# nextpyp/cet_pick

Hardware: AMD Instinct MI355X
Metric: subtomograms/sec (MoCo-3D train) + voxels/sec (heatmap+NMS) at 1/2/4/8 GPU (higher is better)
Workload: dtype f32; 1 GPU; moco_main.py moco3d_18: 3D encoder, synthetic 512x512x128 tomogram, 32^3 subtomo crops, batch 64 per GPU, r=1024, dim=128, m=0.999, T=0.1, SGD lr 1e-3; global_batch=64, parallelism=dp1, hipgraph=True

## Files before the change

### cet_pick_amd/csrc/train_ops.hip

```cpp
#include "common.h"
#include "bf16x3.h"
#include <algorithm>

namespace {

using bf3::ld4;
using bf3::st4;

enum { CR_STATS = 0, CR_BNBWD = 1, CR_SUM = 2, CR_BNBWD_X = 3 };

struct PoolGeom { int N, Di, Hi, Wi, Do, Ho, Wo, k, s, pad; };

struct ColReduceParams {
    const float* a;
    const float* x;
    const float* y;
    const float* save;
    long M;
    int C, relu;
    double* partials;
    const float* gamma;
    const float* beta;
    double* sums_direct;
    float* f32_direct;
// ... 41 lines not shown
            float4 x4 = ld4(p.x + o);
            float x[4] = {x4.x, x4.y, x4.z, x4.w};
            if (p.relu) {
                float4 y4 = ld4(p.y + o);
                float y[4] = {y4.x, y4.y, y4.z, y4.w};
#pragma unroll
                for (int i = 0; i < 4; ++i) a[i] = y[i] > 0.f ? a[i] : 0.f;
            }
#pragma unroll
            for (int i = 0; i < 4; ++i) { s0[i] += a[i]; s1[i] = fmaf(a[i], (x[i] - mean[i]) * inv[i], s1[i]); }
        } else {
#pragma unroll
            for (int i = 0; i < 4; ++i) s0[i] += a[i];
        }
    }
    __shared__ double red[2][256][4];
#pragma unroll
    for (int i = 0; i < 4; ++i) {
        red[0][threadIdx.x][i] = MODE == CR_STATS ? w0[i] : (double)s0[i];
        red[1][threadIdx.x][i] = MODE == CR_STATS ? w1[i] : (double)s1[i];
    }
    __syncthreads();
    if (trow == 0) {
        double a0[4] = {0, 0, 0, 0}, a1[4] = {0, 0, 0, 0};
        for (int rr = 0; rr < RS; ++rr)
#pragma unroll
            for (int i = 0; i < 4; ++i) { a0[i] += red[0][rr * CV + tcol][i]; a1[i] += red[1][rr * CV + tcol][i]; }
        double* dst = p.sums_direct ? p.sums_direct : p.partials + (long)blockIdx.x * 2 * p.C;
#pragma unroll
        for (int i = 0; i < 4; ++i) {
            dst[4 * tcol + i] = a0[i]; dst[p.C + 4 * tcol + i] = a1[i];
            if (p.f32_direct) {
                if (4 * tcol + i < p.n_f32) p.f32_direct[4 * tcol + i] = (float)a0[i];
                if (p.C + 4 * tcol + i < p.n_f32) p.f32_direct[p.C + 4 * tcol + i] = (float)a1[i];
            }
        }
    }
}

__global__ __launch_bounds__(256) void colreduce_finalize_kernel(const double* partials, int n_part,
                                                                int C, double* sums, float* sums_f32, int n_f32) {
    const int c = blockIdx.x * 8 + (threadIdx.x >> 5), l = threadIdx.x & 31;
    double s = 0;
    if (c < 2 * C) {
        int b = l;
        for (; b + 7 * 32 < n_part; b += 8 * 32) {
            double v[8];
#pragma unroll
            for (int u = 0; u < 8; ++u) v[u] = partials[(long)(b + 32 * u) * 2 * C + c];
#pragma unroll
            for (int u = 0; u < 8; ++u) s += v[u];
        }
        for (; b < n_part; b += 32) s += partials[(long)b * 2 * C + c];
    }
#pragma unroll
    for (int o = 16; o > 0; o >>= 1) s += __shfl_xor(s, o, 32);
    if (l == 0 && c < 2 * C) {
        sums[c] = s;
        if (sums_f32 && c < n_f32) sums_f32[c] = (float)s;
    }
}

int colreduce_blocks(long M, int C) {
    int RS = 256 / (C / 4);
    long b = (M + (long)RS * 8 - 1) / ((long)RS * 8);
    long cap = 512;
    if (const char* v = getenv("MI_COLREDUCE_BLOCKS")) { const long cv = atol(v); if (cv >= 1 && cv <= 4096) cap = cv; }
    return (int)std::max<long>(1, std::min<long>(b, cap));
}
bool colreduce_ok(int C) { return C >= 4 && (C % 4) == 0 && (C / 4) <= 256 && (256 % (C / 4)) == 0; }

template <int MODE>
int run_colreduce(ColReduceParams p, double* sums, void* ws, size_t ws_bytes, hipStream_t s, float* sums_f32 = nullptr,
                  int n_f32 = 0) {
    if (!colreduce_ok(p.C) || p.M <= 0) return MI_E_ARG;
    int blocks = colreduce_blocks(p.M, p.C);
    if (!ws || ws_bytes < sizeof(double) * 2 * p.C * (size_t)blocks) return MI_E_WORKSPACE;
    p.partials = (double*)ws;
    if (blocks == 1) {
        p.sums_direct = sums; p.f32_direct = sums_f32; p.n_f32 = n_f32;
        hipLaunchKernelGGL((colreduce_kernel<MODE>), dim3(1), dim3(256), 0, s, p);
        MI_RETURN_IF_LAUNCH_FAILED();
        return MI_OK;
    }
    hipLaunchKernelGGL((colreduce_kernel<MODE>), dim3(blocks), dim3(256), 0, s, p);
    MI_RETURN_IF_LAUNCH_FAILED();
    hipLaunchKernelGGL(colreduce_finalize_kernel, dim3((2 * p.C + 7) / 8), dim3(256), 0, s,
                       (const double*)ws, blocks, p.C, sums, sums_f32, n_f32);
    MI_RETURN_IF_LAUNCH_FAILED();
    return MI_OK;
}

struct BnStat4 { float mean[4], inv[4]; double var[4]; };
__device__ __forceinline__ BnStat4 bn_stat4(const double* sums, double count, int C, int c, float eps) {
    BnStat4 r;
#pragma unroll
    for (int k = 0; k < 4; ++k) {
        const double mean = sums[c + k] / count;
        double var = sums[C + c + k] / count - mean * mean;
        if (var < 0) var = 0;
        r.mean[k] = (float)mean;
        r.inv[k] = (float)(1.0 / sqrt(var + (double)eps));
        r.var[k] = var;
    }
    return r;
}

__global__ __launch_bounds__(256) void bn_apply_kernel(const float* x, float* y, long n4, int C,
                                                      const double* sums, double count, float eps,
                                                      float momentum, float* running_mean,
                                                      float* running_var, long long* num_batches_tracked,
                                                      float* save, const float* gamma,
                                                      const float* beta, const float* res, int relu) {
    const int CV = C >> 2;
    const int c = (int)(threadIdx.x % CV) * 4;
    float m[4], iv[4];
    if (sums) {
        const BnStat4 st = bn_stat4(sums, count, C, c, eps);
#pragma unroll
        for (int k = 0; k < 4; ++k) { m[k] = st.mean[k]; iv[k] = st.inv[k]; }
        if (blockIdx.x == 0 && threadIdx.x < CV) {
#pragma unroll
            for (int k = 0; k < 4; ++k) {
                if (save) { save[c + k] = m[k]; save[C + c + k] = iv[k]; }
                if (running_mean) {
                    const double unbiased = count > 1 ? st.var[k] * count / (count - 1.0) : st.var[k];
                    running_mean[c + k] = (1.f - momentum) * running_mean[c + k] + momentum * m[k];
                    running_var[c + k] = (1.f - momentum) * running_var[c + k] + momentum * (float)unbiased;
                }
            }
            if (threadIdx.x == 0 && num_batches_tracked) *num_batches_tracked += 1;
        }
    } else {
#pragma unroll
        for (int k = 0; k < 4; ++k) { m[k] = running_mean[c + k]; iv[k] = 1.0f / sqrtf(running_var[c + k] + eps); }
        if (save && blockIdx.x == 0 && threadIdx.x < CV) {
#pragma unroll
            for (int k = 0; k < 4; ++k) { save[c + k] = m[k]; save[C + c + k] = iv[k]; }
        }
    }
    const float4 g = gamma ? ld4(gamma + c) : make_float4(1, 1, 1, 1);
    const float4 b = beta ? ld4(beta + c) : make_float4(0, 0, 0, 0);
    for (long i = (long)blockIdx.x * 256 + threadIdx.x; i < n4; i += (long)gridDim.x * 256) {
        float4 v = ld4(x + 4 * i);
        float4 o;
        o.x = fmaf((v.x - m[0]) * iv[0], g.x, b.x); o.y = fmaf((v.y - m[1]) * iv[1], g.y, b.y);
        o.z = fmaf((v.z - m[2]) * iv[2], g.z, b.z); o.w = fmaf((v.w - m[3]) * iv[3], g.w, b.w);
        if (res) { float4 r = ld4(res + 4 * i); o.x += r.x; o.y += r.y; o.z += r.z; o.w += r.w; }
        if (relu) { o.x = fmaxf(o.x, 0.f); o.y = fmaxf(o.y, 0.f); o.z = fmaxf(o.z, 0.f); o.w = fmaxf(o.w, 0.f); }
        st4(y + 4 * i, o);
    }
}

__global__ __launch_bounds__(256) void bn_relu_maxpool_fwd_kernel(const float* x, float* y, uint8_t* arg, PoolGeom g,
                                                                 int C, const double* sums, double count, float eps,
                                                                 float momentum, float* running_mean,
                                                                 float* running_var, long long* num_batches_tracked,
                                                                 float* save, const float* gamma, const float* beta) {
    const int CV = C >> 2;
    const int c = (int)(threadIdx.x % CV) * 4;
    float m[4], iv[4];
    if (sums) {
        const BnStat4 st = bn_stat4(sums, count, C, c, eps);
#pragma unroll
        for (int k = 0; k < 4; ++k) { m[k] = st.mean[k]; iv[k] = st.inv[k]; }
        if (blockIdx.x == 0 && threadIdx.x < CV) {
#pragma unroll
            for (int k = 0; k < 4; ++k) {
                if (save) { save[c + k] = m[k]; save[C + c + k] = iv[k]; }
                if (running_mean) {
                    const double unbiased = count > 1 ? st.var[k] * count / (count - 1.0) : st.var[k];
                    running_mean[c + k] = (1.f - momentum) * running_mean[c + k] + momentum * m[k];
                    running_var[c + k] = (1.f - momentum) * running_var[c + k] + momentum * (float)unbiased;
                }
            }
            if (threadIdx.x == 0 && num_batches_tracked) *num_batches_tracked += 1;
        }
    } else {
#pragma unroll
        for (int k = 0; k < 4; ++k) { m[k] = running_mean[c + k]; iv[k] = 1.0f / sqrtf(running_var[c + k] + eps); }
    }
    const float4 g4 = gamma ? ld4(gamma + c) : make_float4(1, 1, 1, 1);
    const float4 b4 = beta ? ld4(beta + c) : make_float4(0, 0, 0, 0);
    const float gg[4] = {g4.x, g4.y, g4.z, g4.w}, bb[4] = {b4.x, b4.y, b4.z, b4.w};
    const long total = (long)g.N * g.Do * g.Ho * g.Wo * CV;
    for (long i = (long)blockIdx.x * 256 + threadIdx.x; i < total; i += (long)gridDim.x * 256) {
        unsigned v = (unsigned)i / (unsigned)CV;
        const int xo = (int)(v % (unsigned)g.Wo); v /= (unsigned)g.Wo;
        const int yo = (int)(v % (unsigned)g.Ho); v /= (unsigned)g.Ho;
        const int zo = (int)(v % (unsigned)g.Do);
        const int n = (int)(v / (unsigned)g.Do);
        float best[4] = {-INFINITY, -INFINITY, -INFINITY, -INFINITY};
        int bi[4] = {0, 0, 0, 0};
        bool first = true;
        if (g.k == 3) {
            for (int a = 0; a < 3; ++a) {
                const int zi = zo * g.s - g.pad + a;
                const bool zok = (unsigned)zi < (unsigned)g.Di;
                float4 t9[9];
                bool ok9[9];
#pragma unroll
                for (int q = 0; q < 9; ++q) {
                    const int yi = yo * g.s - g.pad + q / 3, xi = xo * g.s - g.pad + q % 3;
                    ok9[q] = zok & ((unsigned)yi < (unsigned)g.Hi) & ((unsigned)xi < (unsigned)g.Wi);
                    const int zc = min(max(zi, 0), g.Di - 1), yc = min(max(yi, 0), g.Hi - 1), xc = min(max(xi, 0), g.Wi - 1);
                    t9[q] = ld4(x + ((((long)n * g.Di + zc) * g.Hi + yc) * g.Wi + xc) * C + c);
                }
#pragma unroll
                for (int q = 0; q < 9; ++q) {
                    if (!ok9[q]) continue;
                    const float xv[4] = {t9[q].x, t9[q].y, t9[q].z, t9[q].w};
                    const int tap = a * 9 + q;
#pragma unroll
                    for (int r = 0; r < 4; ++r) {
                        const float t = fmaxf(fmaf((xv[r] - m[r]) * iv[r], gg[r], bb[r]), 0.f);
                        const float tn = xv[r] != xv[r] ? xv[r] : t;
                        if (first || tn > best[r] || tn != tn) { best[r] = tn; bi[r] = tap; }
                    }
                    first = false;
                }
            }
        } else
        for (int a = 0; a < g.k; ++a) {
            const int zi = zo * g.s - g.pad + a;
            if ((unsigned)zi >= (unsigned)g.Di) continue;
            for (int b = 0; b < g.k; ++b) {
                const int yi = yo * g.s - g.pad + b;
                if ((unsigned)yi >= (unsigned)g.Hi) continue;
                for (int cc = 0; cc < g.k; ++cc) {
                    const int xi = xo * g.s - g.pad + cc;
                    if ((unsigned)xi >= (unsigned)g.Wi) continue;
                    const float4 t4 = ld4(x + ((((long)n * g.Di + zi) * g.Hi + yi) * g.Wi + xi) * C + c);
                    const float xv[4] = {t4.x, t4.y, t4.z, t4.w};
                    const int tap = (a * g.k + b) * g.k + cc;
#pragma unroll
                    for (int q = 0; q < 4; ++q) {
                        const float t = fmaxf(fmaf((xv[q] - m[q]) * iv[q], gg[q], bb[q]), 0.f);
                        const float tn = xv[q] != xv[q] ? xv[q] : t;
                        if (first || tn > best[q] || tn != tn) { best[q] = tn; bi[q] = tap; }
                    }
                    first = false;
                }
            }
        }
        st4(y + 4 * i, make_float4(best[0], best[1], best[2], best[3]));
        if (arg) *reinterpret_cast<uchar4*>(arg + 4 * i) = make_uchar4(bi[0], bi[1], bi[2], bi[3]);
    }
}

__global__ __launch_bounds__(256) void bn_relu_bwd_apply_x_kernel(const float* dy, const float* x, float* dx, long n4, int C,
                                                                 const float* save, const float* gamma, const float* beta,
                                                                 const double* sums, double count, float* dgamma,
                                                                 float* dbeta) {
    const int CV = C >> 2;
    const int c = (int)(threadIdx.x % CV) * 4;
    const float rc = (float)(1.0 / count);
    float mean[4], inv[4], gi[4], gg[4], bb[4], sdy[4], sdx[4];
#pragma unroll
    for (int k = 0; k < 4; ++k) {
        mean[k] = save[c + k]; inv[k] = save[C + c + k];
        gg[k] = gamma ? gamma[c + k] : 1.f; bb[k] = beta ? beta[c + k] : 0.f;
        gi[k] = gg[k] * inv[k];
        sdy[k] = (float)sums[c + k] * rc; sdx[k] = (float)sums[C + c + k] * rc;
    }
    if (blockIdx.x == 0 && threadIdx.x < CV) {
#pragma unroll
        for (int k = 0; k < 4; ++k) {
            if (dbeta) dbeta[c + k] = (float)sums[c + k];
            if (dgamma) dgamma[c + k] = (float)sums[C + c + k];
        }
    }
    for (long i = (long)blockIdx.x * 256 + threadIdx.x; i < n4; i += (long)gridDim.x * 256) {
        const float4 d4 = ld4(dy + 4 * i), x4 = ld4(x + 4 * i);
        const float d[4] = {d4.x, d4.y, d4.z, d4.w}, xv[4] = {x4.x, x4.y, x4.z, x4.w};
        float o[4];
#pragma unroll
        for (int k = 0; k < 4; ++k) {
            const float xh = (xv[k] - mean[k]) * inv[k];
            const float dm = fmaf(xh, gg[k], bb[k]) > 0.f ? d[k] : 0.f;
            o[k] = gi[k] * (dm - sdy[k] - xh * sdx[k]);
        }
        st4(dx + 4 * i, make_float4(o[0], o[1], o[2], o[3]));
    }
}

constexpr int BNS_CH = 4;

__device__ __forceinline__ void bns_block_sum8(double (&v)[8], double (*red)[8]) {
#pragma unroll
    for (int k = 0; k < 8; ++k)
#pragma unroll
        for (int o = 32; o > 0; o >>= 1) v[k] += __shfl_xor(v[k], o, 64);
    const int wave = threadIdx.x >> 6;
    if ((threadIdx.x & 63) == 0)
#pragma unroll
        for (int k = 0; k < 8; ++k) red[wave][k] = v[k];
    __syncthreads();
#pragma unroll
    for (int k = 0; k < 8; ++k) v[k] = (red[0][k] + red[1][k]) + (red[2][k] + red[3][k]);
}

__global__ __launch_bounds__(256) void bn_small_fwd_kernel(const float* x, float* y, int M, int C, const float* gamma,
                                                          const float* beta, float eps, float momentum,
                                                          float* running_mean, float* running_var,
                                                          long long* num_batches_tracked, float* save,
                                                          const float* res, int relu, float* pooled, int V) {
    const int c = blockIdx.x * BNS_CH;
    __shared__ double red[4][8];
    double s[8] = {0, 0, 0, 0, 0, 0, 0, 0};
#pragma unroll 4
    for (int r = threadIdx.x; r < M; r += 256) {
        const float4 v = ld4(x + (long)r * C + c);
        const float a[4] = {v.x, v.y, v.z, v.w};
#pragma unroll
        for (int k = 0; k < 4; ++k) { s[k] += (double)a[k]; s[4 + k] += (double)a[k] * (double)a[k]; }
    }
    bns_block_sum8(s, red);
    float m[4], iv[4];
#pragma unroll
    for (int k = 0; k < 4; ++k) {
        const double mean = s[k] / M;
        double var = s[4 + k] / M - mean * mean;
        if (var < 0) var = 0;
        m[k] = (float)mean; iv[k] = (float)(1.0 / sqrt(var + (double)eps));
        if (threadIdx.x == 0) {
            if (save) { save[c + k] = m[k]; save[C + c + k] = iv[k]; }
            if (running_mean) {
                const double unbiased = M > 1 ? var * M / (M - 1.0) : var;
                running_mean[c + k] = (1.f - momentum) * running_mean[c + k] + momentum * m[k];
                running_var[c + k] = (1.f - momentum) * running_var[c + k] + momentum * (float)unbiased;
            }
        }
    }
    if (blockIdx.x == 0 && threadIdx.x == 0 && num_batches_tracked) *num_batches_tracked += 1;
    const float4 g = gamma ? ld4(gamma + c) : make_float4(1, 1, 1, 1);
    const float4 b = beta ? ld4(beta + c) : make_float4(0, 0, 0, 0);
    if (pooled) {
        const int lane = threadIdx.x & 63;
        for (int r0 = 0; r0 < M; r0 += 256) {
            const int r = r0 + threadIdx.x;
            const bool ok = r < M;
            const long o = (long)(ok ? r : 0) * C + c;
            const float4 v = ld4(x + o);
            float q[4];
            q[0] = fmaf((v.x - m[0]) * iv[0], g.x, b.x); q[1] = fmaf((v.y - m[1]) * iv[1], g.y, b.y);
            q[2] = fmaf((v.z - m[2]) * iv[2], g.z, b.z); q[3] = fmaf((v.w - m[3]) * iv[3], g.w, b.w);
            if (relu) { q[0] = fmaxf(q[0], 0.f); q[1] = fmaxf(q[1], 0.f); q[2] = fmaxf(q[2], 0.f); q[3] = fmaxf(q[3], 0.f); }
            if (ok) st4(y + o, make_float4(q[0], q[1], q[2], q[3]));
            float acc[4] = {q[0], q[1], q[2], q[3]};
            for (int k = 1; k < V; ++k)
#pragma unroll
                for (int e = 0; e < 4; ++e) acc[e] += __shfl(q[e], (lane & ~(V - 1)) + k, 64);
            if (ok && (lane & (V - 1)) == 0) {
                const float rs = (float)V;
                st4(pooled + (long)(r / V) * C + c, make_float4(acc[0] / rs, acc[1] / rs, acc[2] / rs, acc[3] / rs));
            }
        }
        return;
    }
#pragma unroll 4
    for (int r = threadIdx.x; r < M; r += 256) {
        const long o = (long)r * C + c;
        const float4 v = ld4(x + o);
        float4 q;
        q.x = fmaf((v.x - m[0]) * iv[0], g.x, b.x); q.y = fmaf((v.y - m[1]) * iv[1], g.y, b.y);
        q.z = fmaf((v.z - m[2]) * iv[2], g.z, b.z); q.w = fmaf((v.w - m[3]) * iv[3], g.w, b.w);
        if (res) { const float4 t = ld4(res + o); q.x += t.x; q.y += t.y; q.z += t.z; q.w += t.w; }
        if (relu) { q.x = fmaxf(q.x, 0.f); q.y = fmaxf(q.y, 0.f); q.z = fmaxf(q.z, 0.f); q.w = fmaxf(q.w, 0.f); }
        st4(y + o, q);
    }
}

__global__ __launch_bounds__(256) void bn_small_bwd_kernel(const float* dy, const float* x, const float* y, float* dx,
                                                          int M, int C, const float* save, const float* gamma,
                                                          int relu, float* dgamma, float* dbeta, int V) {
    const int c = blockIdx.x * BNS_CH;
    __shared__ double red[4][8];
    const float4 ma = ld4(save + c), ia = ld4(save + C + c);
    const float mean[4] = {ma.x, ma.y, ma.z, ma.w}, inv[4] = {ia.x, ia.y, ia.z, ia.w};
    double s[8] = {0, 0, 0, 0, 0, 0, 0, 0};
#pragma unroll 4
    for (int r = threadIdx.x; r < M; r += 256) {
        const long o = (long)r * C + c;
        const float4 x4 = ld4(x + o);
        float4 d4 = ld4(dy + (V > 0 ? (long)(r / V) * C + c : o));
        if (V > 0) { const float rs = (float)V; d4.x /= rs; d4.y /= rs; d4.z /= rs; d4.w /= rs; }
        float d[4] = {d4.x, d4.y, d4.z, d4.w};
        const float xv[4] = {x4.x, x4.y, x4.z, x4.w};
        if (relu) {
            const float4 y4 = ld4(y + o);
            const float yv[4] = {y4.x, y4.y, y4.z, y4.w};
#pragma unroll
            for (int k = 0; k < 4; ++k) d[k] = yv[k] > 0.f ? d[k] : 0.f;
        }
#pragma unroll
        for (int k = 0; k < 4; ++k) { s[k] += (double)d[k]; s[4 + k] += (double)(d[k] * ((xv[k] - mean[k]) * inv[k])); }
    }
    bns_block_sum8(s, red);
    if (threadIdx.x == 0) {
// ... 371 lines not shown

__device__ unsigned g_ce0_arrivals = 0;
__device__ __forceinline__ bool ce0_split(float lse) { return fabsf(lse) >= 32.f; }
__global__ __launch_bounds__(256) void ce0_rows_kernel(const float* logits, float* loss, float* loss_copy, float* row_loss,
                                                      float* row_lse, int B, int n, unsigned* counter) {
    __shared__ float red[4];
    __shared__ unsigned s_ticket;
    const int b = blockIdx.x, tid = threadIdx.x;
    const float* l = logits + (long)b * n;
    float m = -INFINITY;
    for (int j = tid; j < n; j += 256) m = fmaxf(m, l[j]);
    m = wave_max(m);
    if ((tid & 63) == 0) red[tid >> 6] = m;
    __syncthreads();
    m = fmaxf(fmaxf(red[0], red[1]), fmaxf(red[2], red[3]));
    __syncthreads();
    float s = 0.f;
    for (int j = tid; j < n; j += 256) s += expf(l[j] - m);
    s = wave_sum(s);
    if ((tid & 63) == 0) red[tid >> 6] = s;
    __syncthreads();
    if (tid == 0) {
        const float ls = logf(red[0] + red[1] + red[2] + red[3]);
        const float lse = m + ls;
        row_lse[b] = m;
        row_lse[B + b] = ls;
        __hip_atomic_store(&row_loss[b], ce0_split(lse) ? (m - l[0]) + ls : lse - l[0], __ATOMIC_RELAXED,
                           __HIP_MEMORY_SCOPE_AGENT);
        __builtin_amdgcn_fence(__ATOMIC_RELEASE, "agent");
        asm volatile("s_waitcnt vmcnt(0)" ::: "memory");
        s_ticket = atomicAdd(counter ? counter : &g_ce0_arrivals, 1u);
    }
    __syncthreads();
    if (s_ticket == (unsigned)B - 1 && tid == 0) {
        __builtin_amdgcn_fence(__ATOMIC_ACQUIRE, "agent");
        float t = 0.f;
        for (int r = 0; r < B; ++r) t += __hip_atomic_load(&row_loss[r], __ATOMIC_RELAXED, __HIP_MEMORY_SCOPE_AGENT);
        *loss = t / (float)B;
        if (loss_copy) *loss_copy = t / (float)B;
        __hip_atomic_store(counter ? counter : &g_ce0_arrivals, 0u, __ATOMIC_RELAXED, __HIP_MEMORY_SCOPE_AGENT);
    }
}
__global__ __launch_bounds__(256) void ce0_bwd_kernel(const float* logits, const float* row_lse, const float* g_dev,
                                                     float* dlogits, int B, int n) {
    const int b = blockIdx.x;
    const float g = (*g_dev) / (float)B, m = row_lse[b], ls = row_lse[B + b], lse = m + ls;
    const bool split = ce0_split(lse);
    const float* l = logits + (long)b * n;
    for (int j = threadIdx.x; j < n; j += 256) {
        const float e = split ? expf((l[j] - m) - ls) : expf(l[j] - lse);
        dlogits[(long)b * n + j] = g * (e - (j == 0 ? 1.f : 0.f));
    }
}

__global__ __launch_bounds__(256) void ema_kernel(float* k, const float* q, float m, long n) {
    const float om = 1.0f - m;
    long n4 = n >> 2;
    for (long i = (long)blockIdx.x * 256 + threadIdx.x; i < n4; i += (long)gridDim.x * 256) {
        float4 a = ld4(k + 4 * i), b = ld4(q + 4 * i);
        a.x = a.x * m + b.x * om; a.y = a.y * m + b.y * om;
        a.z = a.z * m + b.z * om; a.w = a.w * m + b.w * om;
        st4(k + 4 * i, a);
    }
    if (blockIdx.x == 0)
        for (long i = (n4 << 2) + threadIdx.x; i < n; i += 256) k[i] = k[i] * m + q[i] * om;
}
__global__ __launch_bounds__(256) void sgd_kernel(float* p, const float* g, const float* lr_dev,
                                                 float lr_host, float wd, float gs, long n) {
    const float lr = lr_dev ? *lr_dev : lr_host;
    long n4 = n >> 2;
    for (long i = (long)blockIdx.x * 256 + threadIdx.x; i < n4; i += (long)gridDim.x * 256) {
        float4 a = ld4(p + 4 * i), b = ld4(g + 4 * i);
        a.x -= lr * (gs * b.x + wd * a.x); a.y -= lr * (gs * b.y + wd * a.y);
        a.z -= lr * (gs * b.z + wd * a.z); a.w -= lr * (gs * b.w + wd * a.w);
        st4(p + 4 * i, a);
    }
    if (blockIdx.x == 0)
        for (long i = (n4 << 2) + threadIdx.x; i < n; i += 256) p[i] -= lr * (gs * g[i] + wd * p[i]);
}

__global__ void enqueue_kernel(float* queue, long long* ptr, const float* keys, int B, int C, int R) {
    const long long p0 = *ptr;
    for (int i = blockIdx.x * blockDim.x + threadIdx.x; i < B * C; i += gridDim.x * blockDim.x) {
        int b = i % B, c = i / B;
        long long col = p0 + b;
        if (col < R) queue[(long)c * R + col] = keys[(long)b * C + c];
    }
}
__global__ void advance_ptr_kernel(long long* ptr, int B, int R) { *ptr = (*ptr + B) % R; }
__global__ __launch_bounds__(1024) void enqueue_small_kernel(float* queue, long long* ptr, const float* keys, int B, int C, int R) {
    const long long p0 = *ptr;
    for (int i = threadIdx.x; i < B * C; i += 1024) {
        int b = i % B, c = i / B;
        long long col = p0 + b;
        if (col < R) queue[(long)c * R + col] = keys[(long)b * C + c];
    }
    __syncthreads();
    if (threadIdx.x == 0) *ptr = (p0 + B) % R;
}

int ew_blocks(long n) { return (int)std::max<long>(1, std::min<long>((n + 255) / 256, 2048)); }

}

extern "C" size_t mi_colreduce_workspace_bytes(long M, int C) {
    if (!colreduce_ok(C)) return 0;
    return sizeof(double) * 2 * C * (size_t)colreduce_blocks(M, C);
}

extern "C" int mi_bn_stats(const float* x, long M, int C, double* sums, void* ws, size_t ws_bytes,
                           mi_stream_t stream) {
    if (!x || !sums) return MI_E_ARG;
    ColReduceParams p = {};
    p.a = x; p.M = M; p.C = C;
    return run_colreduce<CR_STATS>(p, sums, ws, ws_bytes, (hipStream_t)stream);
}

extern "C" int mi_bn_apply_fwd(const float* x, float* y, long M, int C, const double* sums,
                               double count, const float* gamma, const float* beta, float eps,
                               float momentum, float* running_mean, float* running_var,
                               long long* num_batches_tracked, float* save_mean_invstd, const float* res,
                               int relu, mi_stream_t stream) {
    if (!x || !y || !sums || !save_mean_invstd || !colreduce_ok(C) || M <= 0 || !(count > 0)) return MI_E_ARG;
    if ((running_mean == nullptr) != (running_var == nullptr)) return MI_E_ARG;
    hipStream_t s = (hipStream_t)stream;
    long n4 = M * C / 4;
    hipLaunchKernelGGL(bn_apply_kernel, dim3(ew_blocks(n4)), dim3(256), 0, s, x, y, n4, C, sums, count, eps,
                       momentum, running_mean, running_var, num_batches_tracked, save_mean_invstd, gamma,
                       beta, res, relu);
    MI_RETURN_IF_LAUNCH_FAILED();
    return MI_OK;
}

static bool pool_geom(int N, int Di, int Hi, int Wi, int k, int stride, int pad, PoolGeom* g) {
    if (N <= 0 || Di <= 0 || Hi <= 0 || Wi <= 0 || k <= 0 || k > 6 || stride <= 0 || pad < 0) return false;
    if (Di + 2 * pad < k || Hi + 2 * pad < k || Wi + 2 * pad < k) return false;
    const int Do = (Di + 2 * pad - k) / stride + 1, Ho = (Hi + 2 * pad - k) / stride + 1, Wo = (Wi + 2 * pad - k) / stride + 1;
    if (Do <= 0 || Ho <= 0 || Wo <= 0) return false;
    *g = PoolGeom{N, Di, Hi, Wi, Do, Ho, Wo, k, stride, pad};
    return true;
}

extern "C" int mi_bn_relu_maxpool3d_fwd(const float* x, float* y, uint8_t* argmax, int N, int Di, int Hi, int Wi, int C,
                                        int k, int stride, int pad, const double* sums, double count,
                                        const float* gamma, const float* beta, float eps, float momentum,
                                        float* running_mean, float* running_var, long long* num_batches_tracked,
                                        float* save_mean_invstd, mi_stream_t stream) {
    PoolGeom g;
    if (!x || !y || !colreduce_ok(C) || !pool_geom(N, Di, Hi, Wi, k, stride, pad, &g)) return MI_E_ARG;
    if (sums ? (!save_mean_invstd || !(count > 0)) : (!running_mean || !running_var)) return MI_E_ARG;
    if ((running_mean == nullptr) != (running_var == nullptr)) return MI_E_ARG;
    const long total = (long)N * g.Do * g.Ho * g.Wo * (C / 4);
    if (total >= (1l << 31)) return MI_E_UNSUPPORTED;
    hipLaunchKernelGGL(bn_relu_maxpool_fwd_kernel, dim3(ew_blocks(total)), dim3(256), 0, (hipStream_t)stream, x, y, argmax,
                       g, C, sums, count, eps, momentum, running_mean, running_var, num_batches_tracked,
                       save_mean_invstd, gamma, beta);
    MI_RETURN_IF_LAUNCH_FAILED();
    return MI_OK;
}

extern "C" int mi_bn_relu_bwd_reduce_x(const float* dy, const float* x, long M, int C, const float* save_mean_invstd,
                                       const float* gamma, const float* beta, double* sums, void* ws, size_t ws_bytes,
                                       mi_stream_t stream) {
    if (!dy || !x || !save_mean_invstd || !sums) return MI_E_ARG;
    ColReduceParams p = {};
    p.a = dy; p.x = x; p.save = save_mean_invstd; p.M = M; p.C = C; p.gamma = gamma; p.beta = beta;
    return run_colreduce<CR_BNBWD_X>(p, sums, ws, ws_bytes, (hipStream_t)stream);
}

extern "C" int mi_bn_relu_bwd_apply_x(const float* dy, const float* x, float* dx, long M, int C,
                                      const float* save_mean_invstd, const float* gamma, const float* beta,
                                      const double* sums, double count, float* dgamma, float* dbeta, mi_stream_t stream) {
    if (!dy || !x || !dx || !save_mean_invstd || !sums || !colreduce_ok(C) || M <= 0 || !(count > 0)) return MI_E_ARG;
    const long n4 = M * C / 4;
    hipLaunchKernelGGL(bn_relu_bwd_apply_x_kernel, dim3(ew_blocks(n4)), dim3(256), 0, (hipStream_t)stream, dy, x, dx, n4, C,
                       save_mean_invstd, gamma, beta, sums, count, dgamma, dbeta);
    MI_RETURN_IF_LAUNCH_FAILED();
    return MI_OK;
}

extern "C" int mi_bn_small_fwd(const float* x, float* y, long M, int C, const float* gamma, const float* beta,
                               float eps, float momentum, float* running_mean, float* running_var,
                               long long* num_batches_tracked, float* save_mean_invstd, const float* res, int relu,
                               mi_stream_t stream) {
    if (!x || !y || !save_mean_invstd || M <= 0 || M > MI_BN_SMALL_MAX_ROWS || C <= 0 || C % 4) return MI_E_ARG;
    if ((running_mean == nullptr) != (running_var == nullptr)) return MI_E_ARG;
    hipLaunchKernelGGL(bn_small_fwd_kernel, dim3((C + BNS_CH - 1) / BNS_CH), dim3(256), 0, (hipStream_t)stream, x, y,
                       (int)M, C, gamma, beta, eps, momentum, running_mean, running_var, num_batches_tracked,
                       save_mean_invstd, res, relu, (float*)nullptr, 0);
    MI_RETURN_IF_LAUNCH_FAILED();
    return MI_OK;
}

extern "C" int mi_bn_small_pool_fwd(const float* x, float* y, float* pooled, long M, int C, int V, const float* gamma,
                                    const float* beta, float eps, float momentum, float* running_mean, float* running_var,
                                    long long* num_batches_tracked, float* save_mean_invstd, mi_stream_t stream) {
    if (!x || !y || !pooled || !save_mean_invstd || M <= 0 || M > MI_BN_SMALL_MAX_ROWS || C <= 0 || C % 4) return MI_E_ARG;
    if (V < 1 || V > 64 || (V & (V - 1)) || M % V) return MI_E_ARG;
    if ((running_mean == nullptr) != (running_var == nullptr)) return MI_E_ARG;
    hipLaunchKernelGGL(bn_small_fwd_kernel, dim3((C + BNS_CH - 1) / BNS_CH), dim3(256), 0, (hipStream_t)stream, x, y,
                       (int)M, C, gamma, beta, eps, momentum, running_mean, running_var, num_batches_tracked,
                       save_mean_invstd, (const float*)nullptr, 1, pooled, V);
    MI_RETURN_IF_LAUNCH_FAILED();
    return MI_OK;
}

extern "C" int mi_bn_small_bwd(const float* dy, const float* x, const float* y, float* dx, long M, int C,
                               const float* save_mean_invstd, const float* gamma, int relu, float* dgamma,
                               float* dbeta, mi_stream_t stream) {
    if (!dy || !x || !dx || !save_mean_invstd || (relu && !y) || M <= 0 || M > MI_BN_SMALL_MAX_ROWS || C <= 0 || C % 4)
        return MI_E_ARG;
    hipLaunchKernelGGL(bn_small_bwd_kernel, dim3((C + BNS_CH - 1) / BNS_CH), dim3(256), 0, (hipStream_t)stream, dy, x, y,
                       dx, (int)M, C, save_mean_invstd, gamma, relu, dgamma, dbeta, 0);
    MI_RETURN_IF_LAUNCH_FAILED();
    return MI_OK;
}

extern "C" int mi_bn_small_pool_bwd(const float* dpooled, const float* x, const float* y, float* dx, long M, int C, int V,
                                    const float* save_mean_invstd, const float* gamma, float* dgamma, float* dbeta,
                                    mi_stream_t stream) {
    if (!dpooled || !x || !y || !dx || !save_mean_invstd || M <= 0 || M > MI_BN_SMALL_MAX_ROWS || C <= 0 || C % 4) return MI_E_ARG;
    if (V < 1 || V > 64 || (V & (V - 1)) || M % V) return MI_E_ARG;
    hipLaunchKernelGGL(bn_small_bwd_kernel, dim3((C + BNS_CH - 1) / BNS_CH), dim3(256), 0, (hipStream_t)stream, dpooled, x, y,
                       dx, (int)M, C, save_mean_invstd, gamma, 1, dgamma, dbeta, V);
    MI_RETURN_IF_LAUNCH_FAILED();
    return MI_OK;
}

extern "C" int mi_bn_eval_fwd(const float* x, float* y, long M, int C, const float* running_mean,
                              const float* running_var, const float* gamma, const float* beta,
                              float eps, float* save_mean_invstd, const float* res, int relu,
                              mi_stream_t stream) {
    if (!x || !y || !running_mean || !running_var || !colreduce_ok(C) || M <= 0) return MI_E_ARG;
    hipStream_t s = (hipStream_t)stream;
    long n4 = M * C / 4;
    hipLaunchKernelGGL(bn_apply_kernel, dim3(ew_blocks(n4)), dim3(256), 0, s, x, y, n4, C,
                       (const double*)nullptr, 1.0, eps, 0.f, (float*)running_mean, (float*)running_var,
                       (long long*)nullptr, save_mean_invstd, gamma, beta, res, relu);
    MI_RETURN_IF_LAUNCH_FAILED();
    return MI_OK;
}

extern "C" int mi_bn_bwd_reduce(const float* dy, const float* x, const float* y, long M, int C,
                                const float* save_mean_invstd, int relu, double* sums, void* ws,
                                size_t ws_bytes, mi_stream_t stream) {
    if (!dy || !x || !save_mean_invstd || !sums || (relu && !y)) return MI_E_ARG;
    ColReduceParams p = {};
    p.a = dy; p.x = x; p.y = y; p.save = save_mean_invstd; p.M = M; p.C = C; p.relu = relu;
    return run_colreduce<CR_BNBWD>(p, sums, ws, ws_bytes, (hipStream_t)stream);
}

extern "C" int mi_bn_bwd_apply(const float* dy, const float* x, const float* y, float* dx, long M,
                               int C, const float* save_mean_invstd, const float* gamma,
                               const double* sums, double count, int relu, float* dgamma,
                               float* dbeta, mi_stream_t stream) {
    if (!dy || !x || !dx || !save_mean_invstd || !sums || (relu && !y) || !colreduce_ok(C) || !(count > 0)) return MI_E_ARG;
    hipStream_t s = (hipStream_t)stream;
    long n4 = M * C / 4;
    hipLaunchKernelGGL(bn_bwd_apply_kernel, dim3(ew_blocks(n4)), dim3(256), 0, s, dy, x, y, dx, n4, C,
                       save_mean_invstd, gamma, sums, count, relu, dgamma, dbeta, (float*)nullptr);
    MI_RETURN_IF_LAUNCH_FAILED();
    return MI_OK;
}

extern "C" int mi_bn_bwd_apply_res(const float* dy, const float* x, const float* y, float* dx, float* dres, long M,
                                   int C, const float* save_mean_invstd, const float* gamma,
                                   const double* sums, double count, float* dgamma, float* dbeta, mi_stream_t stream) {
    if (!dy || !x || !y || !dx || !dres || !save_mean_invstd || !sums || !colreduce_ok(C) || !(count > 0)) return MI_E_ARG;
    long n4 = M * C / 4;
    hipLaunchKernelGGL(bn_bwd_apply_kernel, dim3(ew_blocks(n4)), dim3(256), 0, (hipStream_t)stream, dy, x, y, dx, n4, C,
                       save_mean_invstd, gamma, sums, count, 1, dgamma, dbeta, dres);
    MI_RETURN_IF_LAUNCH_FAILED();
    return MI_OK;
}

extern "C" int mi_bn_param_grads(const double* sums, int C, float* dgamma, float* dbeta, mi_stream_t stream) {
    if (!sums || C <= 0) return MI_E_ARG;
    hipLaunchKernelGGL(bn_param_grad_kernel, dim3((C + 255) / 256), dim3(256), 0, (hipStream_t)stream, sums, C, dgamma, dbeta);
    MI_RETURN_IF_LAUNCH_FAILED();
    return MI_OK;
}

__global__ __launch_bounds__(256) void colsum_any_kernel(const float* dy, long M, int C, float* out) {
    const int c = blockIdx.x * 4 + (threadIdx.x >> 6), lane = threadIdx.x & 63;
    if (c >= C) return;
    double s = 0;
    for (long r = lane; r < M; r += 64) s += (double)dy[r * C + c];
    s = wave_sum(s);
    if (lane == 0) out[c] = (float)s;
}

extern "C" int mi_colsum(const float* dy, long M, int C, float* out, double* sums_scratch, void* ws,
                         size_t ws_bytes, mi_stream_t stream) {
    if (!dy || !out || !sums_scratch) return MI_E_ARG;
    if (!colreduce_ok(C)) {
        if (M <= 0 || C <= 0) return MI_E_ARG;
        hipLaunchKernelGGL(colsum_any_kernel, dim3((C + 3) / 4), dim3(256), 0, (hipStream_t)stream, dy, M, C, out);
        MI_RETURN_IF_LAUNCH_FAILED();
        return MI_OK;
    }
    ColReduceParams p = {};
    p.a = dy; p.M = M; p.C = C;
    return run_colreduce<CR_SUM>(p, sums_scratch, ws, ws_bytes, (hipStream_t)stream, out, C);
}

extern "C" int mi_maxpool3d_fwd(const float* x, float* y, uint8_t* argmax, int N, int Di, int Hi,
                                int Wi, int C, int k, int stride, int pad, mi_stream_t stream) {
    PoolGeom g;
    if (!x || !y || C <= 0 || C % 4 || !pool_geom(N, Di, Hi, Wi, k, stride, pad, &g)) return MI_E_ARG;
// ... 294 lines not shown
```

Measured before the change: 42140 subtomograms/sec.

## Add specialized k3s2 BN-ReLU-maxpool forward kernel with row reuse and lane shuffles

Adds a specialized forward kernel for 3x3x3 stride-2 pad-1 max pooling fused with BN+ReLU, used when the input width is 16 and channels are a multiple of 32. Each wave handles a band of output rows for one (n, zo, channel group). The previous odd input row is carried over between output rows, and the left x-neighbour comes from a lane shuffle instead of being reloaded, so each input element is read and normalized roughly once rather than up to 27 times. This adds an env-controlled band size, a shape-specific code path, and a custom block-to-work mapping.

Result: no change. 42320 subtomograms/sec (median of 6 runs) (+0.4%).

```diff
diff --git a/cet_pick_amd/csrc/train_ops.hip b/cet_pick_amd/csrc/train_ops.hip
--- a/cet_pick_amd/csrc/train_ops.hip
+++ b/cet_pick_amd/csrc/train_ops.hip
@@ -217,6 +217,44 @@
     }
 }
 
+struct BnPool4 { float m[4], iv[4], g[4], b[4]; };
+__device__ __forceinline__ BnPool4 bn_pool_stats4(bool writer, bool counter, int C, int c, const double* sums, double count,
+                                                  float eps, float momentum, float* running_mean, float* running_var,
+                                                  long long* num_batches_tracked, float* save, const float* gamma,
+                                                  const float* beta) {
+    BnPool4 r;
+    if (sums) {
+        const BnStat4 st = bn_stat4(sums, count, C, c, eps);
+#pragma unroll
+        for (int k = 0; k < 4; ++k) { r.m[k] = st.mean[k]; r.iv[k] = st.inv[k]; }
+        if (writer) {
+#pragma unroll
+            for (int k = 0; k < 4; ++k) {
+                if (save) { save[c + k] = r.m[k]; save[C + c + k] = r.iv[k]; }
+                if (running_mean) {
+                    const double unbiased = count > 1 ? st.var[k] * count / (count - 1.0) : st.var[k];
+                    running_mean[c + k] = (1.f - momentum) * running_mean[c + k] + momentum * r.m[k];
+                    running_var[c + k] = (1.f - momentum) * running_var[c + k] + momentum * (float)unbiased;
+                }
+            }
+            if (counter && num_batches_tracked) *num_batches_tracked += 1;
+        }
+    } else {
+#pragma unroll
+        for (int k = 0; k < 4; ++k) { r.m[k] = running_mean[c + k]; r.iv[k] = 1.0f / sqrtf(running_var[c + k] + eps); }
+    }
+    const float4 g4 = gamma ? ld4(gamma + c) : make_float4(1, 1, 1, 1);
+    const float4 b4 = beta ? ld4(beta + c) : make_float4(0, 0, 0, 0);
+    r.g[0] = g4.x; r.g[1] = g4.y; r.g[2] = g4.z; r.g[3] = g4.w;
+    r.b[0] = b4.x; r.b[1] = b4.y; r.b[2] = b4.z; r.b[3] = b4.w;
+    return r;
+}
+
+__device__ __forceinline__ float bn_relu_nan(float xv, float m, float iv, float g, float b) {
+    const float t = fmaxf(fmaf((xv - m) * iv, g, b), 0.f);
+    return xv != xv ? xv : t;
+}
+
 __global__ __launch_bounds__(256) void bn_relu_maxpool_fwd_kernel(const float* x, float* y, uint8_t* arg, PoolGeom g,
                                                                  int C, const double* sums, double count, float eps,
                                                                  float momentum, float* running_mean,
@@ -224,30 +262,10 @@
                                                                  float* save, const float* gamma, const float* beta) {
     const int CV = C >> 2;
     const int c = (int)(threadIdx.x % CV) * 4;
-    float m[4], iv[4];
-    if (sums) {
-        const BnStat4 st = bn_stat4(sums, count, C, c, eps);
-#pragma unroll
-        for (int k = 0; k < 4; ++k) { m[k] = st.mean[k]; iv[k] = st.inv[k]; }
-        if (blockIdx.x == 0 && threadIdx.x < CV) {
-#pragma unroll
-            for (int k = 0; k < 4; ++k) {
-                if (save) { save[c + k] = m[k]; save[C + c + k] = iv[k]; }
-                if (running_mean) {
-                    const double unbiased = count > 1 ? st.var[k] * count / (count - 1.0) : st.var[k];
-                    running_mean[c + k] = (1.f - momentum) * running_mean[c + k] + momentum * m[k];
-                    running_var[c + k] = (1.f - momentum) * running_var[c + k] + momentum * (float)unbiased;
-                }
-            }
-            if (threadIdx.x == 0 && num_batches_tracked) *num_batches_tracked += 1;
-        }
-    } else {
-#pragma unroll
-        for (int k = 0; k < 4; ++k) { m[k] = running_mean[c + k]; iv[k] = 1.0f / sqrtf(running_var[c + k] + eps); }
-    }
-    const float4 g4 = gamma ? ld4(gamma + c) : make_float4(1, 1, 1, 1);
-    const float4 b4 = beta ? ld4(beta + c) : make_float4(0, 0, 0, 0);
-    const float gg[4] = {g4.x, g4.y, g4.z, g4.w}, bb[4] = {b4.x, b4.y, b4.z, b4.w};
+    const bool writer = blockIdx.x == 0 && threadIdx.x < CV;
+    const BnPool4 bn = bn_pool_stats4(writer, writer && threadIdx.x == 0, C, c, sums, count, eps, momentum, running_mean,
+                                      running_var, num_batches_tracked, save, gamma, beta);
+    const float* m = bn.m; const float* iv = bn.iv; const float* gg = bn.g; const float* bb = bn.b;
     const long total = (long)g.N * g.Do * g.Ho * g.Wo * CV;
     for (long i = (long)blockIdx.x * 256 + threadIdx.x; i < total; i += (long)gridDim.x * 256) {
         unsigned v = (unsigned)i / (unsigned)CV;
@@ -278,8 +296,7 @@
                     const int tap = a * 9 + q;
 #pragma unroll
                     for (int r = 0; r < 4; ++r) {
-                        const float t = fmaxf(fmaf((xv[r] - m[r]) * iv[r], gg[r], bb[r]), 0.f);
-                        const float tn = xv[r] != xv[r] ? xv[r] : t;
+                        const float tn = bn_relu_nan(xv[r], m[r], iv[r], gg[r], bb[r]);
                         if (first || tn > best[r] || tn != tn) { best[r] = tn; bi[r] = tap; }
                     }
                     first = false;
@@ -300,8 +317,7 @@
                     const int tap = (a * g.k + b) * g.k + cc;
 #pragma unroll
                     for (int q = 0; q < 4; ++q) {
-                        const float t = fmaxf(fmaf((xv[q] - m[q]) * iv[q], gg[q], bb[q]), 0.f);
-                        const float tn = xv[q] != xv[q] ? xv[q] : t;
+                        const float tn = bn_relu_nan(xv[q], m[q], iv[q], gg[q], bb[q]);
                         if (first || tn > best[q] || tn != tn) { best[q] = tn; bi[q] = tap; }
                     }
                     first = false;
@@ -310,6 +326,101 @@
         }
         st4(y + 4 * i, make_float4(best[0], best[1], best[2], best[3]));
         if (arg) *reinterpret_cast<uchar4*>(arg + 4 * i) = make_uchar4(bi[0], bi[1], bi[2], bi[3]);
+    }
+}
+
+struct PoolRow4 { float v[4]; int i[4]; };
+__device__ __forceinline__ bool pool_takes(float cand, float best) { return cand > best || cand != cand; }
+
+__device__ __forceinline__ PoolRow4 pool_row_x(const float4 ev, const float4 od, bool has_left, const BnPool4& bn) {
+    const float e[4] = {ev.x, ev.y, ev.z, ev.w}, o[4] = {od.x, od.y, od.z, od.w};
+    PoolRow4 r;
+#pragma unroll
+    for (int q = 0; q < 4; ++q) {
+        const float t1 = bn_relu_nan(e[q], bn.m[q], bn.iv[q], bn.g[q], bn.b[q]);
+        const float t2 = bn_relu_nan(o[q], bn.m[q], bn.iv[q], bn.g[q], bn.b[q]);
+        const float t0 = __shfl_up(t2, 8);
+        float best = has_left ? t0 : t1;
+        int bi = has_left ? 0 : 1;
+        if (has_left && pool_takes(t1, best)) { best = t1; bi = 1; }
+        if (pool_takes(t2, best)) { best = t2; bi = 2; }
+        r.v[q] = best; r.i[q] = bi;
+    }
+    return r;
+}
+__device__ __forceinline__ void pool_merge(PoolRow4& best, bool first, const PoolRow4& cand, int base) {
+#pragma unroll
+    for (int q = 0; q < 4; ++q)
+        if (first || pool_takes(cand.v[q], best.v[q])) { best.v[q] = cand.v[q]; best.i[q] = base + cand.i[q]; }
+}
+
+template <bool ARG>
+__global__ __launch_bounds__(256) void bn_relu_maxpool_k3s2_fwd_kernel(const float* __restrict__ x, float* __restrict__ y,
+                                                                      uint8_t* __restrict__ arg, int N, int Di, int Hi, int Do,
+                                                                      int Ho, int C, int band, const double* sums, double count,
+                                                                      float eps, float momentum, float* running_mean,
+                                                                      float* running_var, long long* num_batches_tracked,
+                                                                      float* save, const float* gamma, const float* beta) {
+    constexpr int Wi = 16, Wo = 8;
+    const int lane = threadIdx.x & 63, xo = lane >> 3, cvl = lane & 7;
+    const unsigned G = (unsigned)C >> 5, nbands = (unsigned)((Ho + band - 1) / band);
+    const unsigned q8 = gridDim.x >> 3, r8 = gridDim.x & 7, grp = blockIdx.x & 7;
+    const unsigned wg = (grp < r8 ? grp * (q8 + 1) : r8 * (q8 + 1) + (grp - r8) * q8) + (blockIdx.x >> 3);
+    const unsigned item = wg * 4 + (unsigned)__builtin_amdgcn_readfirstlane((int)(threadIdx.x >> 6));
+    if (item >= (unsigned)N * Do * nbands * G) return;
+    unsigned t = item;
+    const int g = (int)(t % G); t /= G;
+    const int bnd = (int)(t % nbands); t /= nbands;
+    const int zo = (int)(t % (unsigned)Do), n = (int)(t / (unsigned)Do);
+    const int c = (g * 8 + cvl) * 4;
+    const bool writer = item < G && xo == 0;
+    const BnPool4 bn = bn_pool_stats4(writer, writer && item == 0 && cvl == 0, C, c, sums, count, eps, momentum, running_mean,
+                                      running_var, num_batches_tracked, save, gamma, beta);
+    const int yo0 = bnd * band, yo1 = min(Ho, yo0 + band);
+    const long rowf = (long)Wi * C;
+    const bool zok[3] = {zo > 0, true, 2 * zo + 1 < Di};
+    const float* xz[3];
+#pragma unroll
+    for (int a = 0; a < 3; ++a)
+        xz[a] = x + (((long)n * Di + (zok[a] ? 2 * zo - 1 + a : 2 * zo)) * Hi) * rowf + (2 * xo) * C + c;
+    const bool has_left = xo > 0;
+    PoolRow4 col[3] = {};
+    if (yo0 > 0) {
+        float4 v[3][2];
+#pragma unroll
+        for (int a = 0; a < 3; ++a)
+            if (zok[a]) { const float* p = xz[a] + (2 * yo0 - 1) * rowf; v[a][0] = ld4(p); v[a][1] = ld4(p + C); }
+#pragma unroll
+        for (int a = 0; a < 3; ++a)
+            if (zok[a]) col[a] = pool_row_x(v[a][0], v[a][1], has_left, bn);
+    }
+    for (int yo = yo0; yo < yo1; ++yo) {
+        const bool odd_ok = 2 * yo + 1 < Hi;
+        float4 v[3][4];
+#pragma unroll
+        for (int a = 0; a < 3; ++a)
+            if (zok[a]) {
+                const float* p = xz[a] + (2 * yo) * rowf;
+                v[a][0] = ld4(p); v[a][1] = ld4(p + C);
+                if (odd_ok) { v[a][2] = ld4(p + rowf); v[a][3] = ld4(p + rowf + C); }
+            }
+        PoolRow4 best = {};
+        bool firstz = true;
+#pragma unroll
+        for (int a = 0; a < 3; ++a)
+            if (zok[a]) {
+                PoolRow4 pl = col[a];
+                pool_merge(pl, yo == 0, pool_row_x(v[a][0], v[a][1], has_left, bn), 3);
+                if (odd_ok) {
+                    col[a] = pool_row_x(v[a][2], v[a][3], has_left, bn);
+                    pool_merge(pl, false, col[a], 6);
+                }
+                pool_merge(best, firstz, pl, 9 * a);
+                firstz = false;
+            }
+        const long o = ((((long)n * Do + zo) * Ho + yo) * Wo + xo) * C + c;
+        st4(y + o, make_float4(best.v[0], best.v[1], best.v[2], best.v[3]));
+        if (ARG) *reinterpret_cast<uchar4*>(arg + o) = make_uchar4(best.i[0], best.i[1], best.i[2], best.i[3]);
     }
 }
 
@@ -987,9 +1098,23 @@
     if ((running_mean == nullptr) != (running_var == nullptr)) return MI_E_ARG;
     const long total = (long)N * g.Do * g.Ho * g.Wo * (C / 4);
     if (total >= (1l << 31)) return MI_E_UNSUPPORTED;
-    hipLaunchKernelGGL(bn_relu_maxpool_fwd_kernel, dim3(ew_blocks(total)), dim3(256), 0, (hipStream_t)stream, x, y, argmax,
-                       g, C, sums, count, eps, momentum, running_mean, running_var, num_batches_tracked,
-                       save_mean_invstd, gamma, beta);
+    int band = 4;
+    if (const char* v = getenv("MI_BN_POOL_FWD_BAND")) { const int bv = atoi(v); if (bv >= 1 && bv <= 64) band = bv; }
+    if (k == 3 && stride == 2 && pad == 1 && Wi == 16 && C % 32 == 0 && !getenv("MI_BN_POOL_FWD_GENERIC")) {
+        const long waves = (long)N * g.Do * ((g.Ho + band - 1) / band) * (C / 32);
+        const dim3 grid((unsigned)((waves + 3) / 4));
+        if (argmax)
+            hipLaunchKernelGGL(bn_relu_maxpool_k3s2_fwd_kernel<true>, grid, dim3(256), 0, (hipStream_t)stream, x, y, argmax, N, Di,
+                               Hi, g.Do, g.Ho, C, band, sums, count, eps, momentum, running_mean, running_var,
+                               num_batches_tracked, save_mean_invstd, gamma, beta);
+        else
+            hipLaunchKernelGGL(bn_relu_maxpool_k3s2_fwd_kernel<false>, grid, dim3(256), 0, (hipStream_t)stream, x, y, argmax, N,
+                               Di, Hi, g.Do, g.Ho, C, band, sums, count, eps, momentum, running_mean, running_var,
+                               num_batches_tracked, save_mean_invstd, gamma, beta);
+    } else
+        hipLaunchKernelGGL(bn_relu_maxpool_fwd_kernel, dim3(ew_blocks(total)), dim3(256), 0, (hipStream_t)stream, x, y, argmax,
+                           g, C, sums, count, eps, momentum, running_mean, running_var, num_batches_tracked,
+                           save_mean_invstd, gamma, beta);
     MI_RETURN_IF_LAUNCH_FAILED();
     return MI_OK;
 }
```
